# LouisNUST/pose-unsupervised

Hardware: AMD Instinct MI355X
Metric: 4-view 256x256 frames/sec (fwd+triangulate) (higher is better)
Workload: dtype bf16

## Files before the change

### pose-unsupervised_amd/csrc/stem.hip

```cpp
#include <string>
#include <type_traits>

#include "posu_common.h"

namespace posu {
namespace {

constexpr int kStemK = 224;
constexpr int kStemPitch = 232;
typedef unsigned int u32x4 __attribute__((ext_vector_type(4)));

template <typename T>
struct StemOp;
template <>
struct StemOp<uint16_t> {
  static __device__ __forceinline__ void mma(f32x4& acc, const uint4& a, const uint4& b) {
    acc = __builtin_amdgcn_mfma_f32_16x16x32_bf16(__builtin_bit_cast(bf16x8, a), __builtin_bit_cast(bf16x8, b), acc,
                                                  0, 0, 0);
  }
  static __device__ __forceinline__ uint32_t pack2(float a, float b) {
    return f2bf2(a, b);
  }
};
template <>
struct StemOp<f16_t> {
  static __device__ __forceinline__ void mma(f32x4& acc, const uint4& a, const uint4& b) {
    acc = __builtin_amdgcn_mfma_f32_16x16x32_f16(__builtin_bit_cast(f16x8, a), __builtin_bit_cast(f16x8, b), acc, 0,
                                                 0, 0);
  }
  static __device__ __forceinline__ uint32_t pack2(float a, float b) {
    const _Float16 ha = static_cast<_Float16>(a), hb = static_cast<_Float16>(b);
    return static_cast<uint32_t>(__builtin_bit_cast(uint16_t, ha)) |
           (static_cast<uint32_t>(__builtin_bit_cast(uint16_t, hb)) << 16);
  }
};

constexpr int kMaxViews = 8;
struct StemViews {
  const float* x[kMaxViews];
};

#ifndef POSU_STEM_ABLATE
#define POSU_STEM_ABLATE 0
#endif
#ifndef POSU_STEM_PFD
#define POSU_STEM_PFD 1
#endif
constexpr int kStemAbl = POSU_STEM_ABLATE;

template <typename T, int NW, bool SPL = false, bool RAW = false>
__global__ __launch_bounds__(NW * 64, 1) void stem_pool_kernel(StemViews xs, int Nv, int N, int H, int W, int hflip,
                                                               int strips, const void* __restrict__ wv_,
                                                               const float* __restrict__ scale,
                                                               const float* __restrict__ shift, T* __restrict__ y) {
  using O = StemOp<T>;
  constexpr int NT = NW * 64;
  constexpr int WP = NW * 32 + 8;
  constexpr int RB = WP * 8;
  constexpr int RING = 16;
  constexpr int W_BYTES = 64 * kStemPitch * 2;
  constexpr int NS = SPL ? 2 : 1;
  constexpr int CPX = SPL ? 128 : 64;
  static_assert(!SPL || (NW == 8 && std::is_same<T, f16_t>::value), "split stem: fp16 halves, eight waves");
  static_assert(!RAW || (!SPL && NW == 8), "raw stem: one dtype, eight waves");
  const T* __restrict__ w = static_cast<const T*>(wv_);
  __shared__ __attribute__((aligned(16))) char smem[NS * (RING * RB + W_BYTES) + NW * 2 * 64 * 4 + 2 * 64 * 4];
  char* win = smem;
  char* winl = smem + RING * RB;
  char* wl = smem + NS * RING * RB;
  char* wll = wl + W_BYTES;
  float* edge = reinterpret_cast<float*>(smem + NS * (RING * RB + W_BYTES));
  float* bn = edge + NW * 2 * 64;

  const int tid = threadIdx.x, lane = tid & 63, wid = tid >> 6;
  const int r16 = lane & 15, q = lane >> 4;
  const int Hp = H / 4, Wp = W / 4;
  const int pairs = Hp / 2, per = pairs / strips;
  const int n = blockIdx.x / strips;
  const int k0 = (blockIdx.x - n * strips) * per, k1 = k0 + per;
  const float* __restrict__ xn = xs.x[n / Nv] + static_cast<size_t>(n % Nv) * 3 * H * W;
  const size_t plane = static_cast<size_t>(H) * W;

  if constexpr (RAW) {
    const float* __restrict__ wf = static_cast<const float*>(wv_);
    for (int i = tid; i < 64 * kStemK / 2; i += NT) {
      const int co = i / (kStemK / 2), k0 = 2 * (i - co * (kStemK / 2));
      float v[2];
#pragma unroll
      for (int u = 0; u < 2; ++u) {
        const int k = k0 + u, kh = k >> 5, kw = (k >> 2) & 7, ci = k & 3;
        v[u] = (kw < 7 && ci < 3) ? wf[((co * 3 + ci) * 7 + kh) * 7 + kw] : 0.f;
      }
      *reinterpret_cast<uint32_t*>(wl + (co * kStemPitch + k0) * 2) = O::pack2(v[0], v[1]);
    }
  } else {
  if (tid < 64) {
    bn[tid] = fabsf(scale[tid]);
    bn[64 + tid] = shift[tid];
  }
  {
    constexpr int WCH = 64 * (kStemK / 8);
#pragma unroll
    for (int it = 0; it < (NS * WCH + NT - 1) / NT; ++it) {
      const int i = tid + it * NT;
      if (i < NS * WCH) {
        const int h = i / WCH, ii = i - h * WCH;
        const int co = ii / (kStemK / 8), ck = ii - co * (kStemK / 8);
        const unsigned sg = __float_as_uint(scale[co]) & 0x80000000u ? 0x80008000u : 0u;
        u32x4 wv = *reinterpret_cast<const u32x4*>(w + i * 8);
        wv ^= sg;
        *reinterpret_cast<u32x4*>((h ? wll : wl) + (co * kStemPitch + ck * 8) * 2) = wv;
      }
    }
  }
  }

  constexpr int GPR = NW * 8 + 2;
  constexpr int XG8 = (8 * GPR + NT - 1) / NT;
  auto load_rows = [&](int i0, auto nr, float4 (*xv)[3]) __attribute__((always_inline)) {
    constexpr int NR = decltype(nr)::value, XG = (NR * GPR + NT - 1) / NT;
#pragma unroll
    for (int it = 0; it < XG; ++it) {
      const int i = tid + it * NT;
      const int r = i / GPR, gk = i - r * GPR;
      const int iy = i0 + r, c0 = 4 * (gk - 1);
#pragma unroll
      for (int p = 0; p < 3; ++p) xv[it][p] = make_float4(0.f, 0.f, 0.f, 0.f);
      if (kStemAbl & 2) {
        xv[it][0] = make_float4(iy, c0, 1.f, 0.5f);
        continue;
      }
      if (i < NR * GPR && static_cast<unsigned>(iy) < static_cast<unsigned>(H) &&
          static_cast<unsigned>(c0) < static_cast<unsigned>(W)) {
        const size_t o = static_cast<size_t>(iy) * W + (hflip ? W - 4 - c0 : c0);
#pragma unroll
        for (int p = 0; p < 3; ++p) {
          float4 v = *reinterpret_cast<const float4*>(xn + p * plane + o);
          if (hflip) v = make_float4(v.w, v.z, v.y, v.x);
          xv[it][p] = v;
        }
      }
    }
  };
  auto store_rows = [&](int i0, auto nr, float4 (*xv)[3]) __attribute__((always_inline)) {
    constexpr int NR = decltype(nr)::value, XG = (NR * GPR + NT - 1) / NT;
#pragma unroll
    for (int it = 0; it < XG; ++it) {
      const int i = tid + it * NT;
      if (i >= NR * GPR) continue;
      const int r = i / GPR, gk = i - r * GPR;
      char* row = win + ((i0 + r) & (RING - 1)) * RB;
      const float a0[4] = {xv[it][0].x, xv[it][0].y, xv[it][0].z, xv[it][0].w};
      const float a1[4] = {xv[it][1].x, xv[it][1].y, xv[it][1].z, xv[it][1].w};
      const float a2[4] = {xv[it][2].x, xv[it][2].y, xv[it][2].z, xv[it][2].w};
#pragma unroll
      for (int e = 0; e < 4; ++e) {
        const int wc = 4 * gk - 1 + e;
        if (wc >= 0 && wc < WP) {
          *reinterpret_cast<uint2*>(row + wc * 8) = make_uint2(O::pack2(a0[e], a1[e]), O::pack2(a2[e], 0.f));
          if constexpr (SPL) {
            const float l0 = a0[e] - static_cast<float>(static_cast<_Float16>(a0[e]));
            const float l1 = a1[e] - static_cast<float>(static_cast<_Float16>(a1[e]));
            const float l2 = a2[e] - static_cast<float>(static_cast<_Float16>(a2[e]));
            *reinterpret_cast<uint2*>(row - win + winl + wc * 8) = make_uint2(O::pack2(l0, l1), O::pack2(l2, 0.f));
          }
        }
      }
    }
  };

  const int sc = 16 * wid + r16;
  auto stem_rows = [&](int r0, auto mrows, float (*carry)[4], float (*vm)[4][4]) __attribute__((always_inline)) {
    constexpr int M = decltype(mrows)::value;
    f32x4 acc[M][4];
#pragma unroll
    for (int i = 0; i < M; ++i)
#pragma unroll
      for (int j = 0; j < 4; ++j) acc[i][j] = f32x4{0.f, 0.f, 0.f, 0.f};
    auto rd = [&](int rho) {
      return *reinterpret_cast<const uint4*>(win + ((2 * r0 - 3 + rho) & (RING - 1)) * RB + (2 * sc + 2 * q) * 8);
    };
    auto rdl = [&](int rho) {
      return *reinterpret_cast<const uint4*>(winl + ((2 * r0 - 3 + rho) & (RING - 1)) * RB + (2 * sc + 2 * q) * 8);
    };
    auto bload = [&](int kh, uint4 (&bfr)[4]) {
#pragma unroll
      for (int j = 0; j < 4; ++j)
        bfr[j] = *reinterpret_cast<const uint4*>(wl + ((16 * j + r16) * kStemPitch + kh * 32 + 8 * q) * 2);
    };
    auto bloadl = [&](int kh, uint4 (&bfr)[4]) {
#pragma unroll
      for (int j = 0; j < 4; ++j)
        bfr[j] = *reinterpret_cast<const uint4*>(wll + ((16 * j + r16) * kStemPitch + kh * 32 + 8 * q) * 2);
    };
    auto mmas = [&](const uint4 (&bfr)[4], const uint4 (&af)[M]) {
#pragma unroll
      for (int rl = 0; rl < M; ++rl)
#pragma unroll
        for (int j = 0; j < 4; ++j) {
          if (kStemAbl & 1) acc[rl][j][0] += __uint_as_float(bfr[j].x ^ af[rl].y);
          else O::mma(acc[rl][j], bfr[j], af[rl]);
        }
    };
    if constexpr (SPL) {
      uint4 ev[M], od[M], evl[M], odl[M], bfr[4], bfl[4];
#pragma unroll
      for (int kh = 0; kh < 7; ++kh) {
        uint4 (&set)[M] = (kh & 1) ? od : ev;
        uint4 (&setl)[M] = (kh & 1) ? odl : evl;
        bload(kh, bfr);
        bloadl(kh, bfl);
        if (kh < 2) {
#pragma unroll
          for (int rl = 0; rl < M; ++rl) {
            set[rl] = rd(kh + 2 * rl);
            setl[rl] = rdl(kh + 2 * rl);
          }
        } else {
#pragma unroll
          for (int rl = 0; rl + 1 < M; ++rl) {
            set[rl] = set[rl + 1];
            setl[rl] = setl[rl + 1];
          }
          set[M - 1] = rd(kh + 2 * (M - 1));
          setl[M - 1] = rdl(kh + 2 * (M - 1));
        }
        mmas(bfr, set);
        mmas(bfl, set);
        mmas(bfr, setl);
      }
    } else if constexpr (NW <= 8) {
      uint4 ev[M], od[M], bfr[4];
#pragma unroll
      for (int kh = 0; kh < 7; ++kh) {
        uint4 (&set)[M] = (kh & 1) ? od : ev;
        bload(kh, bfr);
        if (kh < 2) {
#pragma unroll
          for (int rl = 0; rl < M; ++rl) set[rl] = rd(kh + 2 * rl);
        } else {
#pragma unroll
          for (int rl = 0; rl + 1 < M; ++rl) set[rl] = set[rl + 1];
          set[M - 1] = rd(kh + 2 * (M - 1));
        }
        mmas(bfr, set);
      }
    } else {
#pragma unroll 1
      for (int kh = 0; kh < 7; ++kh) {
        uint4 bfr[4];
        bload(kh, bfr);
#pragma unroll
        for (int rl = 0; rl < M; ++rl) {
          const uint4 af = rd(kh + 2 * rl);
#pragma unroll
          for (int j = 0; j < 4; ++j) O::mma(acc[rl][j], bfr[j], af);
        }
      }
    }
    if constexpr (RAW) {
      T* __restrict__ zr = y + (static_cast<size_t>(n) * (H / 2) + r0) * (W / 2) * 64 + sc * 64 + 4 * q;
#pragma unroll
      for (int rl = 0; rl < M; ++rl)
#pragma unroll
        for (int j = 0; j < 4; ++j) {
          const uint2 u = make_uint2(O::pack2(acc[rl][j][0], acc[rl][j][1]), O::pack2(acc[rl][j][2], acc[rl][j][3]));
          if (kStemAbl & 4) asm volatile("" ::"v"(u.x), "v"(u.y));
          else *reinterpret_cast<uint2*>(zr + static_cast<size_t>(rl) * (W / 2) * 64 + 16 * j) = u;
        }
      return;
    }
#pragma unroll
    for (int j = 0; j < 4; ++j)
#pragma unroll
      for (int e = 0; e < 4; ++e) {
        float v[M];
#pragma unroll
        for (int rl = 0; rl < M; ++rl)
          v[rl] = (M == 4 || r0 + rl >= 0) ? acc[rl][j][e] : -INFINITY;
        const float first = M == 5 ? v[0] : carry[j][e];
        const float* u = v + (M == 5 ? 1 : 0);
        vm[0][j][e] = fmaxf(fmaxf(first, u[0]), u[1]);
        vm[1][j][e] = fmaxf(fmaxf(u[1], u[2]), u[3]);
        carry[j][e] = u[3];
      }
  };

  T* __restrict__ yn = y + static_cast<size_t>(n) * Hp * Wp * CPX;
  auto pool = [&](int k, const float (*vm)[4][4]) __attribute__((always_inline)) {
    if (r16 == 15) {
#pragma unroll
      for (int p = 0; p < 2; ++p)
#pragma unroll
        for (int j = 0; j < 4; ++j)
          *reinterpret_cast<float4*>(edge + (wid * 2 + p) * 64 + 16 * j + 4 * q) =
              make_float4(vm[p][j][0], vm[p][j][1], vm[p][j][2], vm[p][j][3]);
    }
    __syncthreads();
    const int wl = wid > 0 ? wid - 1 : 0;
    const bool first_col = r16 == 0, pad_left = wid == 0;
#pragma unroll
    for (int p = 0; p < 2; ++p)
#pragma unroll
      for (int j = 0; j < 4; ++j) {
        const float4 s4 = *reinterpret_cast<const float4*>(bn + 16 * j + 4 * q);
        const float4 b4 = *reinterpret_cast<const float4*>(bn + 64 + 16 * j + 4 * q);
        const float sv[4] = {s4.x, s4.y, s4.z, s4.w}, bv[4] = {b4.x, b4.y, b4.z, b4.w};
        const float4 l4 = *reinterpret_cast<const float4*>(edge + (wl * 2 + p) * 64 + 16 * j + 4 * q);
        const float lv[4] = {l4.x, l4.y, l4.z, l4.w};
        float o[4];
#pragma unroll
        for (int e = 0; e < 4; ++e) {
          const float self = vm[p][j][e];
          const float right = __int_as_float(__builtin_amdgcn_update_dpp(0, __float_as_int(self), 0x101, 0xf, 0xf, true));
          float left = __int_as_float(__builtin_amdgcn_update_dpp(0, __float_as_int(self), 0x111, 0xf, 0xf, true));
          if (first_col) left = pad_left ? -INFINITY : lv[e];
          o[e] = fmaxf(fmaf(sv[e], fmaxf(fmaxf(left, self), right), bv[e]), 0.f);
        }
        if ((r16 & 1) == 0) {
          const int pc = 8 * wid + (r16 >> 1);
          const int c0 = 16 * j + 4 * q;
          T* dst = yn + (static_cast<size_t>(2 * k + p) * Wp + pc) * CPX + (SPL ? split_ch(c0) : c0);
          const uint2 u = make_uint2(O::pack2(o[0], o[1]), O::pack2(o[2], o[3]));
          if (kStemAbl & 4) {
            asm volatile("" ::"v"(u.x), "v"(u.y));
          } else {
            *reinterpret_cast<uint2*>(dst) = u;
            if constexpr (SPL) {
              float l[4];
#pragma unroll
              for (int e = 0; e < 4; ++e) l[e] = o[e] - static_cast<float>(static_cast<_Float16>(o[e]));
              *reinterpret_cast<uint2*>(dst + 32) = make_uint2(O::pack2(l[0], l[1]), O::pack2(l[2], l[3]));
            }
          }
        }
      }
  };

  using I4 = std::integral_constant<int, 4>;
  using I5 = std::integral_constant<int, 5>;
  using I8 = std::integral_constant<int, 8>;
  float carry[4][4], vm[2][4][4];
  constexpr bool PF = NW <= 8;
  constexpr int PFD = PF ? POSU_STEM_PFD : 1;
  static_assert(PFD == 1 || PFD == 2, "prefetch depth 1 or 2");
  float4 xv[PFD][XG8][3];
  load_rows(8 * k0 - 5, I8{}, xv[0]);
  store_rows(8 * k0 - 5, I8{}, xv[0]);
  load_rows(8 * k0 + 3, I8{}, xv[0]);
  store_rows(8 * k0 + 3, I8{}, xv[0]);
  __syncthreads();
  if constexpr (RAW) stem_rows(4 * k0, I4{}, carry, vm);
  else stem_rows(4 * k0 - 1, I5{}, carry, vm);
  if constexpr (PF) {
    if (k0 + 1 < k1) load_rows(8 * k0 + 10, I8{}, xv[PFD - 1]);
    if (PFD == 2 && k0 + 2 < k1) load_rows(8 * k0 + 18, I8{}, xv[0]);
  }
  if constexpr (RAW) __syncthreads();
  else pool(k0, vm);
  auto item = [&](int k, auto sidx) __attribute__((always_inline)) {
    constexpr int S = decltype(sidx)::value;
    if (!PF) load_rows(8 * k + 2, I8{}, xv[S]);
    store_rows(8 * k + 2, I8{}, xv[S]);
    __syncthreads();
    if (PF && k + PFD < k1) load_rows(8 * (k + PFD) + 2, I8{}, xv[S]);
    if constexpr (PF) stem_rows(4 * k, I4{}, carry, vm);
    else stem_rows(4 * k - 1, I5{}, carry, vm);
    if constexpr (RAW) {
      __syncthreads();
    } else {
      pool(k, vm);
    }
  };
  using S0 = std::integral_constant<int, 0>;
  using S1 = std::integral_constant<int, PFD - 1>;
  int k = k0 + 1;
  if constexpr (PFD == 2) {
    for (; k + 1 < k1; k += 2) {
      item(k, S1{});
      item(k + 1, S0{});
    }
  }
  for (; k < k1; ++k) item(k, S1{});
}


typedef short s16x4 __attribute__((ext_vector_type(4)));
constexpr int kWgThreads = 448;
constexpr int kWgRing = 16;
constexpr int kWgCols = 264;
constexpr int kWgRB = kWgCols * 8;
constexpr int kWgDz = 128 * 128;
constexpr int kWgGroups = 66;
constexpr int kWgPart = 7 * 32 * 64;

__device__ __forceinline__ int wg_sw(int px) { return (((px >> 1) & 1) << 1) | (((px >> 3) & 1) << 2); }

__device__ __forceinline__ uint4 tr_pair(const char* p0, const char* p1) {
  const s16x4 v0 = __builtin_amdgcn_ds_read_tr16_b64_v4i16((__attribute__((address_space(3))) s16x4*)(p0));
  const s16x4 v1 = __builtin_amdgcn_ds_read_tr16_b64_v4i16((__attribute__((address_space(3))) s16x4*)(p1));
  const uint2 u0 = __builtin_bit_cast(uint2, v0), u1 = __builtin_bit_cast(uint2, v1);
  return make_uint4(u0.x, u0.y, u1.x, u1.y);
}

template <typename T>
__global__ __launch_bounds__(kWgThreads, 2) void stem_wgrad_kernel(StemViews xs, int Nv, int H, int strips,
                                                                   const T* __restrict__ dz, float* __restrict__ part) {
  using O = StemOp<T>;
  constexpr int W = 256, Wo = 128;
  __shared__ __attribute__((aligned(16))) char smem[kWgRing * kWgRB + 2 * kWgDz];
  char* ring = smem;
  char* dzb = smem + kWgRing * kWgRB;
  const int tid = threadIdx.x, lane = tid & 63, kh = tid >> 6;
  const int q = lane >> 4, a = (lane >> 2) & 3, p = lane & 3;
  const int Ho = H / 2, rows = Ho / strips;
  const int n = blockIdx.x / strips;
  const int ya = (blockIdx.x - n * strips) * rows, yb = ya + rows;
  const float* __restrict__ xn = xs.x[n / Nv] + static_cast<size_t>(n % Nv) * 3 * H * W;
  const size_t plane = static_cast<size_t>(H) * W;
  const T* __restrict__ dzn = dz + static_cast<size_t>(n) * Ho * Wo * 64;

  auto load_x = [&](int iy0, int nr, int it, float4 (&xv)[3]) {
    const int i = tid + it * kWgThreads;
    const int r = i / kWgGroups, g = i - r * kWgGroups;
    const int iy = iy0 + r, c0 = 4 * (g - 1);
    const bool ok = i < nr * kWgGroups && static_cast<unsigned>(iy) < static_cast<unsigned>(H) &&
                    static_cast<unsigned>(c0) < static_cast<unsigned>(W);
    const size_t o = ok ? static_cast<size_t>(iy) * W + c0 : 0;
#pragma unroll
    for (int pl = 0; pl < 3; ++pl) {
      const float4 v = *reinterpret_cast<const float4*>(xn + pl * plane + o);
      xv[pl] = ok ? v : make_float4(0.f, 0.f, 0.f, 0.f);
    }
  };
  auto store_x = [&](int iy0, int nr, int it, const float4 (&xv)[3]) {
    const int i = tid + it * kWgThreads;
    if (i >= nr * kWgGroups) return;
    const int r = i / kWgGroups, g = i - r * kWgGroups;
    char* row = ring + ((iy0 + r) & (kWgRing - 1)) * kWgRB;
    auto cmp = [](const float4& v, int e) { return e == 0 ? v.x : e == 1 ? v.y : e == 2 ? v.z : v.w; };
#pragma unroll
    for (int e = 0; e < 4; ++e) {
      const int wc = 4 * g - 1 + e;
      if (wc >= 0 && wc < kWgCols)
        *reinterpret_cast<uint2*>(row + wc * 8) =
            make_uint2(O::pack2(cmp(xv[0], e), cmp(xv[1], e)), O::pack2(cmp(xv[2], e), 0.f));
    }
  };
  auto load_dz = [&](int oy, uint4 (&dv)[3]) {
#pragma unroll
    for (int it = 0; it < 3; ++it) {
      const int i = tid + it * kWgThreads;
      dv[it] = i < 1024 ? *reinterpret_cast<const uint4*>(dzn + (static_cast<size_t>(oy) * Wo) * 64 + i * 8)
                        : make_uint4(0, 0, 0, 0);
    }
  };
  auto store_dz = [&](int buf, const uint4 (&dv)[3]) {
#pragma unroll
    for (int it = 0; it < 3; ++it) {
      const int i = tid + it * kWgThreads;
      if (i < 1024) {
        const int px = i >> 3, c = i & 7;
        *reinterpret_cast<uint4*>(dzb + buf * kWgDz + px * 128 + ((c ^ wg_sw(px)) << 4)) = dv[it];
      }
    }
  };

  {
    float4 xv[3];
#pragma unroll
    for (int it = 0; it < (7 * kWgGroups + kWgThreads - 1) / kWgThreads; ++it) {
      load_x(2 * ya - 3, 7, it, xv);
      store_x(2 * ya - 3, 7, it, xv);
    }
    uint4 dv[3];
    load_dz(ya, dv);
    store_dz(0, dv);
  }
  __syncthreads();

  f32x4 acc[4][2];
#pragma unroll
  for (int mt = 0; mt < 4; ++mt)
#pragma unroll
    for (int hf = 0; hf < 2; ++hf) acc[mt][hf] = f32x4{0.f, 0.f, 0.f, 0.f};
  for (int oy = ya; oy < yb; ++oy) {
    const bool more = oy + 1 < yb;
    float4 xv[3];
    uint4 dv[3];
    if (more) {
      load_x(2 * oy + 4, 2, 0, xv);
      load_dz(oy + 1, dv);
    }
    const char* dzr = dzb + (oy & 1) * kWgDz;
    const char* xr = ring + ((2 * oy - 3 + kh) & (kWgRing - 1)) * kWgRB;
#pragma unroll
    for (int s = 0; s < 4; ++s) {
      const int px0 = 32 * s + 8 * q + a, px1 = px0 + 4;
      uint4 af[4], bf[2];
#pragma unroll
      for (int mt = 0; mt < 4; ++mt) {
        const int chunk = 2 * mt + (p >> 1), within = (p & 1) * 8;
        af[mt] = tr_pair(dzr + px0 * 128 + ((chunk ^ wg_sw(px0)) << 4) + within,
                         dzr + px1 * 128 + ((chunk ^ wg_sw(px1)) << 4) + within);
      }
#pragma unroll
      for (int hf = 0; hf < 2; ++hf)
        bf[hf] = tr_pair(xr + 16 * px0 + 32 * hf + 8 * p, xr + 16 * px1 + 32 * hf + 8 * p);
#pragma unroll
      for (int mt = 0; mt < 4; ++mt)
#pragma unroll
        for (int hf = 0; hf < 2; ++hf) {
          if (kStemAbl & 1) acc[mt][hf][0] += __uint_as_float(af[mt].x ^ bf[hf].y);
          else O::mma(acc[mt][hf], af[mt], bf[hf]);
        }
    }
    if (more) {
      store_x(2 * oy + 4, 2, 0, xv);
      store_dz((oy + 1) & 1, dv);
    }
    __syncthreads();
  }
  float* dst = part + static_cast<size_t>(blockIdx.x) * kWgPart + kh * 32 * 64;
#pragma unroll
  for (int mt = 0; mt < 4; ++mt)
#pragma unroll
    for (int hf = 0; hf < 2; ++hf)
      *reinterpret_cast<float4*>(dst + (16 * hf + (lane & 15)) * 64 + 16 * mt + 4 * q) =
          make_float4(acc[mt][hf][0], acc[mt][hf][1], acc[mt][hf][2], acc[mt][hf][3]);
}

constexpr int kWrLanes = 16;
__global__ __launch_bounds__(256) void stem_wgrad_reduce_kernel(const float* __restrict__ part, int nblocks,
                                                                 float* __restrict__ dw) {
  __shared__ float red[kWrLanes][17];
  const int c = threadIdx.x & 15, sl = threadIdx.x >> 4;
  const int rest = blockIdx.x >> 2, co = (blockIdx.x & 3) * 16 + c;
  const int ci = rest % 3, tap = rest / 3, kh = tap / 7, kw = tap - 7 * kh;
  const float* p = part + (kh * 32 + kw * 4 + ci) * 64 + co;
  float s = 0.f;
#pragma unroll 4
  for (int b = sl; b < nblocks; b += kWrLanes) s += p[static_cast<size_t>(b) * kWgPart];
  red[sl][c] = s;
  __syncthreads();
  if (threadIdx.x < 16) {
    float t = 0.f;
#pragma unroll
    for (int l = 0; l < kWrLanes; ++l) t += red[l][threadIdx.x];
    dw[((co * 3 + ci) * 7 + kh) * 7 + kw] = t;
  }
}

}
}

using namespace posu;

namespace {
int stem_launch(int dtype, const float* const* views, int nviews, int Nv, int H, int W, int hflip, const void* w,
                const float* scale, const float* shift, void* y, void* stream, const char* what) {
  const std::string wh(what);
  POSU_REQUIRE(dtype == POSU_BF16 || dtype == POSU_F16 || dtype == POSU_F16X3, wh + ": dtype must be BF16, F16 or F16X3");
  POSU_REQUIRE(dtype != POSU_F16X3 || W == 256, wh + ": the split-fp16 stem is built for W = 256");
  POSU_REQUIRE(views && nviews >= 1 && nviews <= kMaxViews, wh + ": 1 .. 8 views");
  for (int v = 0; v < nviews; ++v) POSU_REQUIRE(views[v], wh + ": null view pointer");
  POSU_REQUIRE(w && scale && shift && y, wh + ": null pointer");
  POSU_REQUIRE(Nv > 0 && H > 0 && H % 8 == 0 && (W == 256 || W == 384),
               wh + ": needs H % 8 == 0 and W in {256, 384}");
  POSU_REQUIRE(static_cast<long long>(Nv) * 3 * H * W < (1LL << 40), wh + ": input too large");
  StemViews xs{};
  for (int v = 0; v < nviews; ++v) xs.x[v] = views[v];
  const int N = Nv * nviews, pairs = H / 8;
  int strips = 1;
  while (N * strips * 2 <= 256 && pairs % (strips * 2) == 0) strips *= 2;
  hipStream_t s = as_stream(stream);
  const dim3 grid(static_cast<unsigned>(N * strips));
  if (dtype == POSU_F16X3) {
    hipLaunchKernelGGL((stem_pool_kernel<f16_t, 8, true>), grid, dim3(512), 0, s, xs, Nv, N, H, W, hflip, strips,
                       static_cast<const f16_t*>(w), scale, shift, static_cast<f16_t*>(y));
  } else if (dtype == POSU_BF16) {
    if (W == 256)
      hipLaunchKernelGGL((stem_pool_kernel<uint16_t, 8>), grid, dim3(512), 0, s, xs, Nv, N, H, W, hflip, strips,
                         static_cast<const uint16_t*>(w), scale, shift, static_cast<uint16_t*>(y));
    else
      hipLaunchKernelGGL((stem_pool_kernel<uint16_t, 12>), grid, dim3(768), 0, s, xs, Nv, N, H, W, hflip, strips,
                         static_cast<const uint16_t*>(w), scale, shift, static_cast<uint16_t*>(y));
  } else {
    if (W == 256)
      hipLaunchKernelGGL((stem_pool_kernel<f16_t, 8>), grid, dim3(512), 0, s, xs, Nv, N, H, W, hflip, strips,
                         static_cast<const f16_t*>(w), scale, shift, static_cast<f16_t*>(y));
    else
      hipLaunchKernelGGL((stem_pool_kernel<f16_t, 12>), grid, dim3(768), 0, s, xs, Nv, N, H, W, hflip, strips,
                         static_cast<const f16_t*>(w), scale, shift, static_cast<f16_t*>(y));
  }
  return check_launch(what);
}
}

extern "C" int posu_stem_pool_fwd(int dtype, const float* x, int N, int H, int W, int hflip, const void* w,
                                  const float* scale, const float* shift, void* y, void* stream) {
  return stem_launch(dtype, &x, 1, N, H, W, hflip, w, scale, shift, y, stream, "posu_stem_pool_fwd");
}

extern "C" int posu_stem_pool_views_fwd(int dtype, const float* const* views, int nviews, int Nv, int H, int W,
                                        int hflip, const void* w, const float* scale, const float* shift, void* y,
                                        void* stream) {
  return stem_launch(dtype, views, nviews, Nv, H, W, hflip, w, scale, shift, y, stream, "posu_stem_pool_views_fwd");
}

namespace {
int stem_train_views(const char* what, int dtype, const float* const* views, int nviews, int Nv, int H, int W,
                     StemViews& xs) {
  const std::string wh(what);
  POSU_REQUIRE(dtype == POSU_BF16 || dtype == POSU_F16, wh + ": dtype must be BF16 or F16");
  POSU_REQUIRE(views && nviews >= 1 && nviews <= kMaxViews, wh + ": 1 .. 8 views");
  for (int v = 0; v < nviews; ++v) POSU_REQUIRE(views[v], wh + ": null view pointer");
  POSU_REQUIRE(Nv > 0 && H > 0 && H % 8 == 0 && W == 256, wh + ": built for W = 256 and H % 8 == 0");
  POSU_REQUIRE(static_cast<long long>(Nv) * 3 * H * W < (1LL << 40), wh + ": input too large");
  for (int v = 0; v < nviews; ++v) {
    POSU_REQUIRE((reinterpret_cast<size_t>(views[v]) & 15) == 0, wh + ": views must be 16-byte aligned");
    xs.x[v] = views[v];
  }
  return 0;
}

int wgrad_strips(int N, int H) {
  int strips = 1;
  while (N * strips * 2 <= 512 && (H / 2) % (strips * 2) == 0 && (H / 2) / (strips * 2) >= 8) strips *= 2;
  return strips;
}
}

extern "C" int posu_stem_conv_views_fwd(int dtype, const float* const* views, int nviews, int Nv, int H, int W,
                                        const float* w, void* z, void* stream) {
  StemViews xs{};
  const int rc = stem_train_views("posu_stem_conv_views_fwd", dtype, views, nviews, Nv, H, W, xs);
  if (rc) return rc;
  POSU_REQUIRE(w && z, "posu_stem_conv_views_fwd: null pointer");
  const int N = Nv * nviews, pairs = H / 8;
  int strips = 1;
  while (N * strips * 2 <= 256 && pairs % (strips * 2) == 0) strips *= 2;
  hipStream_t s = as_stream(stream);
  const dim3 grid(static_cast<unsigned>(N * strips));
  if (dtype == POSU_BF16)
    hipLaunchKernelGGL((stem_pool_kernel<uint16_t, 8, false, true>), grid, dim3(512), 0, s, xs, Nv, N, H, W, 0, strips,
                       static_cast<const void*>(w), nullptr, nullptr, static_cast<uint16_t*>(z));
  else
    hipLaunchKernelGGL((stem_pool_kernel<f16_t, 8, false, true>), grid, dim3(512), 0, s, xs, Nv, N, H, W, 0, strips,
                       static_cast<const void*>(w), nullptr, nullptr, static_cast<f16_t*>(z));
  return check_launch("posu_stem_conv_views_fwd");
}

extern "C" long long posu_stem_wgrad_workspace(int N, int H, int W) {
  if (N <= 0 || H <= 0 || H % 8 != 0 || W != 256) return -1;
  return static_cast<long long>(N) * wgrad_strips(N, H) * kWgPart * 4;
}

extern "C" int posu_stem_wgrad_views(int dtype, const float* const* views, int nviews, int Nv, int H, int W,
                                     const void* dz, float* dw, void* workspace, long long workspace_bytes,
                                     void* stream) {
  StemViews xs{};
  const int rc = stem_train_views("posu_stem_wgrad_views", dtype, views, nviews, Nv, H, W, xs);
  if (rc) return rc;
  POSU_REQUIRE(dz && dw && workspace, "posu_stem_wgrad_views: null pointer");
  POSU_REQUIRE((reinterpret_cast<size_t>(dz) & 15) == 0 && (reinterpret_cast<size_t>(workspace) & 15) == 0,
               "posu_stem_wgrad_views: dz / workspace must be 16-byte aligned");
  const int N = Nv * nviews, strips = wgrad_strips(N, H);
  POSU_REQUIRE(workspace_bytes >= posu_stem_wgrad_workspace(N, H, W), "posu_stem_wgrad_views: workspace too small");
  hipStream_t s = as_stream(stream);
  float* part = static_cast<float*>(workspace);
  const dim3 grid(static_cast<unsigned>(N * strips));
  if (dtype == POSU_BF16)
    hipLaunchKernelGGL(stem_wgrad_kernel<uint16_t>, grid, dim3(kWgThreads), 0, s, xs, Nv, H, strips,
                       static_cast<const uint16_t*>(dz), part);
  else
    hipLaunchKernelGGL(stem_wgrad_kernel<f16_t>, grid, dim3(kWgThreads), 0, s, xs, Nv, H, strips,
                       static_cast<const f16_t*>(dz), part);
  hipLaunchKernelGGL(stem_wgrad_reduce_kernel, dim3(147 * 4), dim3(256), 0, s, part, N * strips, dw);
  return check_launch("posu_stem_wgrad_views");
}
```

Baseline: 56430.

## Process one pooled row per stem item with two blocks per CU

Adds a PR=1 variant of the fused stem conv+maxpool kernel that handles a single pooled row per iteration instead of two. It launches with a two-blocks-per-CU launch bound and twice as many strips (up to 512 blocks) so that more waves are resident. It double-buffers the edge exchange buffer to drop one barrier per item, pads the left edge with a -inf sentinel so the boundary branch goes away, and hoists the BN loads. The trade-off is halved register/LDS budget per block, more per-row overhead and more halo recompute. A debug occupancy query entry point is also added.

```diff
diff --git a/pose-unsupervised_amd/csrc/stem.hip b/pose-unsupervised_amd/csrc/stem.hip
--- a/pose-unsupervised_amd/csrc/stem.hip
+++ b/pose-unsupervised_amd/csrc/stem.hip
@@ -46,36 +46,44 @@
 #ifndef POSU_STEM_PFD
 #define POSU_STEM_PFD 1
 #endif
+#ifndef POSU_STEM_ONEB
+#define POSU_STEM_ONEB 1
+#endif
 constexpr int kStemAbl = POSU_STEM_ABLATE;
 
-template <typename T, int NW, bool SPL = false, bool RAW = false>
-__global__ __launch_bounds__(NW * 64, 1) void stem_pool_kernel(StemViews xs, int Nv, int N, int H, int W, int hflip,
-                                                               int strips, const void* __restrict__ wv_,
-                                                               const float* __restrict__ scale,
-                                                               const float* __restrict__ shift, T* __restrict__ y) {
+template <typename T, int NW, bool SPL = false, bool RAW = false, int PR = 2>
+__global__ __launch_bounds__(NW * 64, PR == 1 ? 2 : 1) void stem_pool_kernel(
+    StemViews xs, int Nv, int N, int H, int W, int hflip, int strips, const void* __restrict__ wv_,
+    const float* __restrict__ scale, const float* __restrict__ shift, T* __restrict__ y) {
   using O = StemOp<T>;
+  static_assert(PR == 2 || (PR == 1 && NW == 8 && !SPL && !RAW), "one-pool-row items: the pooled eight-wave kernel");
   constexpr int NT = NW * 64;
+  constexpr int MR = 2 * PR;
+  constexpr int NRI = 4 * PR;
   constexpr int WP = NW * 32 + 8;
   constexpr int RB = WP * 8;
   constexpr int RING = 16;
   constexpr int W_BYTES = 64 * kStemPitch * 2;
   constexpr int NS = SPL ? 2 : 1;
   constexpr int CPX = SPL ? 128 : 64;
+  constexpr bool ONEB = PR == 1 && POSU_STEM_ONEB;
+  constexpr int NE = ONEB ? 2 : 1;
+  constexpr int ES = (NW + 1) * PR * 64;
   static_assert(!SPL || (NW == 8 && std::is_same<T, f16_t>::value), "split stem: fp16 halves, eight waves");
   static_assert(!RAW || (!SPL && NW == 8), "raw stem: one dtype, eight waves");
   const T* __restrict__ w = static_cast<const T*>(wv_);
-  __shared__ __attribute__((aligned(16))) char smem[NS * (RING * RB + W_BYTES) + NW * 2 * 64 * 4 + 2 * 64 * 4];
+  __shared__ __attribute__((aligned(16))) char smem[NS * (RING * RB + W_BYTES) + NE * ES * 4 + 2 * 64 * 4];
   char* win = smem;
   char* winl = smem + RING * RB;
   char* wl = smem + NS * RING * RB;
   char* wll = wl + W_BYTES;
   float* edge = reinterpret_cast<float*>(smem + NS * (RING * RB + W_BYTES));
-  float* bn = edge + NW * 2 * 64;
+  float* bn = edge + NE * ES;
 
   const int tid = threadIdx.x, lane = tid & 63, wid = tid >> 6;
   const int r16 = lane & 15, q = lane >> 4;
   const int Hp = H / 4, Wp = W / 4;
-  const int pairs = Hp / 2, per = pairs / strips;
+  const int items = Hp / PR, per = items / strips;
   const int n = blockIdx.x / strips;
   const int k0 = (blockIdx.x - n * strips) * per, k1 = k0 + per;
   const float* __restrict__ xn = xs.x[n / Nv] + static_cast<size_t>(n % Nv) * 3 * H * W;
@@ -98,6 +106,7 @@
     bn[tid] = fabsf(scale[tid]);
     bn[64 + tid] = shift[tid];
   }
+  for (int i = tid; i < NE * PR * 64; i += NT) edge[i / (PR * 64) * ES + i % (PR * 64)] = -INFINITY;
   {
     constexpr int WCH = 64 * (kStemK / 8);
 #pragma unroll
@@ -116,7 +125,7 @@
   }
 
   constexpr int GPR = NW * 8 + 2;
-  constexpr int XG8 = (8 * GPR + NT - 1) / NT;
+  constexpr int XGI = (NRI * GPR + NT - 1) / NT;
   auto load_rows = [&](int i0, auto nr, float4 (*xv)[3]) __attribute__((always_inline)) {
     constexpr int NR = decltype(nr)::value, XG = (NR * GPR + NT - 1) / NT;
 #pragma unroll
@@ -277,50 +286,59 @@
         float v[M];
 #pragma unroll
         for (int rl = 0; rl < M; ++rl)
-          v[rl] = (M == 4 || r0 + rl >= 0) ? acc[rl][j][e] : -INFINITY;
-        const float first = M == 5 ? v[0] : carry[j][e];
-        const float* u = v + (M == 5 ? 1 : 0);
-        vm[0][j][e] = fmaxf(fmaxf(first, u[0]), u[1]);
-        vm[1][j][e] = fmaxf(fmaxf(u[1], u[2]), u[3]);
-        carry[j][e] = u[3];
+          v[rl] = (M == MR || r0 + rl >= 0) ? acc[rl][j][e] : -INFINITY;
+        const float first = M == MR + 1 ? v[0] : carry[j][e];
+        const float* u = v + (M == MR + 1 ? 1 : 0);
+#pragma unroll
+        for (int p = 0; p < PR; ++p)
+          vm[p][j][e] = fmaxf(fmaxf(p ? u[2 * p - 1] : first, u[2 * p]), u[2 * p + 1]);
+        carry[j][e] = u[MR - 1];
       }
   };
 
   T* __restrict__ yn = y + static_cast<size_t>(n) * Hp * Wp * CPX;
   auto pool = [&](int k, const float (*vm)[4][4]) __attribute__((always_inline)) {
+    float* eb = edge + (ONEB ? (k & 1) * ES : 0);
+    float4 s4[4], b4[4];
+#pragma unroll
+    for (int j = 0; j < 4; ++j) {
+      s4[j] = *reinterpret_cast<const float4*>(bn + 16 * j + 4 * q);
+      b4[j] = *reinterpret_cast<const float4*>(bn + 64 + 16 * j + 4 * q);
+    }
     if (r16 == 15) {
 #pragma unroll
-      for (int p = 0; p < 2; ++p)
+      for (int p = 0; p < PR; ++p)
 #pragma unroll
         for (int j = 0; j < 4; ++j)
-          *reinterpret_cast<float4*>(edge + (wid * 2 + p) * 64 + 16 * j + 4 * q) =
+          *reinterpret_cast<float4*>(eb + ((wid + 1) * PR + p) * 64 + 16 * j + 4 * q) =
               make_float4(vm[p][j][0], vm[p][j][1], vm[p][j][2], vm[p][j][3]);
     }
     __syncthreads();
-    const int wl = wid > 0 ? wid - 1 : 0;
-    const bool first_col = r16 == 0, pad_left = wid == 0;
-#pragma unroll
-    for (int p = 0; p < 2; ++p)
+    float4 l4[PR][4];
+#pragma unroll
+    for (int p = 0; p < PR; ++p)
+#pragma unroll
+      for (int j = 0; j < 4; ++j)
+        l4[p][j] = *reinterpret_cast<const float4*>(eb + (wid * PR + p) * 64 + 16 * j + 4 * q);
+#pragma unroll
+    for (int p = 0; p < PR; ++p)
 #pragma unroll
       for (int j = 0; j < 4; ++j) {
-        const float4 s4 = *reinterpret_cast<const float4*>(bn + 16 * j + 4 * q);
-        const float4 b4 = *reinterpret_cast<const float4*>(bn + 64 + 16 * j + 4 * q);
-        const float sv[4] = {s4.x, s4.y, s4.z, s4.w}, bv[4] = {b4.x, b4.y, b4.z, b4.w};
-        const float4 l4 = *reinterpret_cast<const float4*>(edge + (wl * 2 + p) * 64 + 16 * j + 4 * q);
-        const float lv[4] = {l4.x, l4.y, l4.z, l4.w};
+        const float sv[4] = {s4[j].x, s4[j].y, s4[j].z, s4[j].w}, bv[4] = {b4[j].x, b4[j].y, b4[j].z, b4[j].w};
+        const float lv[4] = {l4[p][j].x, l4[p][j].y, l4[p][j].z, l4[p][j].w};
         float o[4];
 #pragma unroll
         for (int e = 0; e < 4; ++e) {
           const float self = vm[p][j][e];
           const float right = __int_as_float(__builtin_amdgcn_update_dpp(0, __float_as_int(self), 0x101, 0xf, 0xf, true));
-          float left = __int_as_float(__builtin_amdgcn_update_dpp(0, __float_as_int(self), 0x111, 0xf, 0xf, true));
-          if (first_col) left = pad_left ? -INFINITY : lv[e];
+          const float left =
+              __int_as_float(__builtin_amdgcn_update_dpp(__float_as_int(lv[e]), __float_as_int(self), 0x111, 0xf, 0xf, false));
           o[e] = fmaxf(fmaf(sv[e], fmaxf(fmaxf(left, self), right), bv[e]), 0.f);
         }
         if ((r16 & 1) == 0) {
           const int pc = 8 * wid + (r16 >> 1);
           const int c0 = 16 * j + 4 * q;
-          T* dst = yn + (static_cast<size_t>(2 * k + p) * Wp + pc) * CPX + (SPL ? split_ch(c0) : c0);
+          T* dst = yn + (static_cast<size_t>(PR * k + p) * Wp + pc) * CPX + (SPL ? split_ch(c0) : c0);
           const uint2 u = make_uint2(O::pack2(o[0], o[1]), O::pack2(o[2], o[3]));
           if (kStemAbl & 4) {
             asm volatile("" ::"v"(u.x), "v"(u.y));
@@ -337,35 +355,55 @@
       }
   };
 
-  using I4 = std::integral_constant<int, 4>;
-  using I5 = std::integral_constant<int, 5>;
-  using I8 = std::integral_constant<int, 8>;
-  float carry[4][4], vm[2][4][4];
+  using IM = std::integral_constant<int, MR>;
+  using IM1 = std::integral_constant<int, MR + 1>;
+  using INR = std::integral_constant<int, NRI>;
+  float carry[4][4], vm[PR][4][4];
   constexpr bool PF = NW <= 8;
   constexpr int PFD = PF ? POSU_STEM_PFD : 1;
   static_assert(PFD == 1 || PFD == 2, "prefetch depth 1 or 2");
-  float4 xv[PFD][XG8][3];
-  load_rows(8 * k0 - 5, I8{}, xv[0]);
-  store_rows(8 * k0 - 5, I8{}, xv[0]);
-  load_rows(8 * k0 + 3, I8{}, xv[0]);
-  store_rows(8 * k0 + 3, I8{}, xv[0]);
+  float4 xv[PFD][XGI][3];
+  if constexpr (PR == 1) {
+    float4 x0[3][XGI][3];
+#pragma unroll
+    for (int l = 0; l < 3; ++l) load_rows(NRI * k0 - 5 + NRI * l, INR{}, x0[l]);
+#pragma unroll
+    for (int l = 0; l < 3; ++l) store_rows(NRI * k0 - 5 + NRI * l, INR{}, x0[l]);
+  } else {
+    load_rows(NRI * k0 - 5, INR{}, xv[0]);
+    store_rows(NRI * k0 - 5, INR{}, xv[0]);
+    load_rows(NRI * k0 + NRI - 5, INR{}, xv[0]);
+    store_rows(NRI * k0 + NRI - 5, INR{}, xv[0]);
+  }
   __syncthreads();
-  if constexpr (RAW) stem_rows(4 * k0, I4{}, carry, vm);
-  else stem_rows(4 * k0 - 1, I5{}, carry, vm);
+  if constexpr (ONEB) {
+    if (k0 + 1 < k1) load_rows(NRI * (k0 + 1) + 2, INR{}, xv[0]);
+    stem_rows(MR * k0 - 1, IM1{}, carry, vm);
+    for (int k = k0;;) {
+      if (k + 1 < k1) store_rows(NRI * (k + 1) + 2, INR{}, xv[0]);
+      if (k + 2 < k1) load_rows(NRI * (k + 2) + 2, INR{}, xv[0]);
+      pool(k, vm);
+      if (++k >= k1) break;
+      stem_rows(MR * k, IM{}, carry, vm);
+    }
+    return;
+  }
+  if constexpr (RAW) stem_rows(MR * k0, IM{}, carry, vm);
+  else stem_rows(MR * k0 - 1, IM1{}, carry, vm);
   if constexpr (PF) {
-    if (k0 + 1 < k1) load_rows(8 * k0 + 10, I8{}, xv[PFD - 1]);
-    if (PFD == 2 && k0 + 2 < k1) load_rows(8 * k0 + 18, I8{}, xv[0]);
+    if (k0 + 1 < k1) load_rows(NRI * (k0 + 1) + 2, INR{}, xv[PFD - 1]);
+    if (PFD == 2 && k0 + 2 < k1) load_rows(NRI * (k0 + 2) + 2, INR{}, xv[0]);
   }
   if constexpr (RAW) __syncthreads();
   else pool(k0, vm);
   auto item = [&](int k, auto sidx) __attribute__((always_inline)) {
     constexpr int S = decltype(sidx)::value;
-    if (!PF) load_rows(8 * k + 2, I8{}, xv[S]);
-    store_rows(8 * k + 2, I8{}, xv[S]);
+    if (!PF) load_rows(NRI * k + 2, INR{}, xv[S]);
+    store_rows(NRI * k + 2, INR{}, xv[S]);
     __syncthreads();
-    if (PF && k + PFD < k1) load_rows(8 * (k + PFD) + 2, I8{}, xv[S]);
-    if constexpr (PF) stem_rows(4 * k, I4{}, carry, vm);
-    else stem_rows(4 * k - 1, I5{}, carry, vm);
+    if (PF && k + PFD < k1) load_rows(NRI * (k + PFD) + 2, INR{}, xv[S]);
+    if constexpr (PF) stem_rows(MR * k, IM{}, carry, vm);
+    else stem_rows(MR * k - 1, IM1{}, carry, vm);
     if constexpr (RAW) {
       __syncthreads();
     } else {
@@ -570,9 +608,11 @@
   POSU_REQUIRE(static_cast<long long>(Nv) * 3 * H * W < (1LL << 40), wh + ": input too large");
   StemViews xs{};
   for (int v = 0; v < nviews; ++v) xs.x[v] = views[v];
-  const int N = Nv * nviews, pairs = H / 8;
+  const int N = Nv * nviews;
+  const bool two = dtype != POSU_F16X3 && W == 256;
+  const int items = two ? H / 4 : H / 8, blocks = two ? 512 : 256;
   int strips = 1;
-  while (N * strips * 2 <= 256 && pairs % (strips * 2) == 0) strips *= 2;
+  while (N * strips * 2 <= blocks && items % (strips * 2) == 0) strips *= 2;
   hipStream_t s = as_stream(stream);
   const dim3 grid(static_cast<unsigned>(N * strips));
   if (dtype == POSU_F16X3) {
@@ -580,14 +620,14 @@
                        static_cast<const f16_t*>(w), scale, shift, static_cast<f16_t*>(y));
   } else if (dtype == POSU_BF16) {
     if (W == 256)
-      hipLaunchKernelGGL((stem_pool_kernel<uint16_t, 8>), grid, dim3(512), 0, s, xs, Nv, N, H, W, hflip, strips,
+      hipLaunchKernelGGL((stem_pool_kernel<uint16_t, 8, false, false, 1>), grid, dim3(512), 0, s, xs, Nv, N, H, W, hflip, strips,
                          static_cast<const uint16_t*>(w), scale, shift, static_cast<uint16_t*>(y));
     else
       hipLaunchKernelGGL((stem_pool_kernel<uint16_t, 12>), grid, dim3(768), 0, s, xs, Nv, N, H, W, hflip, strips,
                          static_cast<const uint16_t*>(w), scale, shift, static_cast<uint16_t*>(y));
   } else {
     if (W == 256)
-      hipLaunchKernelGGL((stem_pool_kernel<f16_t, 8>), grid, dim3(512), 0, s, xs, Nv, N, H, W, hflip, strips,
+      hipLaunchKernelGGL((stem_pool_kernel<f16_t, 8, false, false, 1>), grid, dim3(512), 0, s, xs, Nv, N, H, W, hflip, strips,
                          static_cast<const f16_t*>(w), scale, shift, static_cast<f16_t*>(y));
     else
       hipLaunchKernelGGL((stem_pool_kernel<f16_t, 12>), grid, dim3(768), 0, s, xs, Nv, N, H, W, hflip, strips,
@@ -606,6 +646,22 @@
                                         int hflip, const void* w, const float* scale, const float* shift, void* y,
                                         void* stream) {
   return stem_launch(dtype, views, nviews, Nv, H, W, hflip, w, scale, shift, y, stream, "posu_stem_pool_views_fwd");
+}
+
+extern "C" int posu_dbg_stem_pool_blocks_per_cu(int dtype, int W) {
+  int nb = -1;
+  hipError_t e = hipErrorInvalidValue;
+  if (dtype == POSU_F16X3 && W == 256)
+    e = hipOccupancyMaxActiveBlocksPerMultiprocessor(&nb, stem_pool_kernel<f16_t, 8, true>, 512, 0);
+  else if (dtype == POSU_BF16 && W == 256)
+    e = hipOccupancyMaxActiveBlocksPerMultiprocessor(&nb, stem_pool_kernel<uint16_t, 8, false, false, 1>, 512, 0);
+  else if (dtype == POSU_F16 && W == 256)
+    e = hipOccupancyMaxActiveBlocksPerMultiprocessor(&nb, stem_pool_kernel<f16_t, 8, false, false, 1>, 512, 0);
+  else if (dtype == POSU_BF16 && W == 384)
+    e = hipOccupancyMaxActiveBlocksPerMultiprocessor(&nb, stem_pool_kernel<uint16_t, 12>, 768, 0);
+  else if (dtype == POSU_F16 && W == 384)
+    e = hipOccupancyMaxActiveBlocksPerMultiprocessor(&nb, stem_pool_kernel<f16_t, 12>, 768, 0);
+  return e == hipSuccess ? nb : -1;
 }
 
 namespace {
```

After: 56830 (median of 6 runs). No clear change (+0.7%).
